# ruizhecao96/CMGAN

Measured on NVIDIA H100. Metric: utterances/sec (2 s @16 kHz) generator fwd+bwd, higher is better.
Workload: dtype tf32

## Files before the change

cmgan_b200/_lib.py:

```python
from __future__ import annotations

import ctypes
import os
import re

HERE = os.path.dirname(os.path.abspath(__file__))
ROOT = os.path.dirname(HERE)
HEADER = os.path.join(ROOT, "include", "cmgan_b200.h")
LIB_PATH = os.path.join(HERE, "libcmgan_b200.so")
MAX_TAPS = 16


class GemmArgs(ctypes.Structure):
    _fields_ = [
        ("A", ctypes.c_void_p), ("lda", ctypes.c_longlong),
        ("B", ctypes.c_void_p), ("sb_tap", ctypes.c_longlong), ("sb_k", ctypes.c_longlong), ("sb_n", ctypes.c_longlong),
        ("bias", ctypes.c_void_p),
        ("C", ctypes.c_void_p), ("ldc", ctypes.c_longlong),
        ("M", ctypes.c_int), ("N", ctypes.c_int), ("Cin", ctypes.c_int), ("ntaps", ctypes.c_int),
        ("conv", ctypes.c_int), ("OH", ctypes.c_int), ("OW", ctypes.c_int), ("IH", ctypes.c_int), ("IW", ctypes.c_int),
        ("mul_y", ctypes.c_int), ("mul_x", ctypes.c_int), ("div_y", ctypes.c_int), ("div_x", ctypes.c_int),
        ("dy", ctypes.c_int * MAX_TAPS), ("dx", ctypes.c_int * MAX_TAPS),
        ("tap_off", ctypes.c_longlong * MAX_TAPS),
        ("pro", ctypes.c_int), ("pro_alpha", ctypes.c_float), ("p0", ctypes.c_void_p), ("p1", ctypes.c_void_p), ("p2", ctypes.c_void_p),
        ("rows_per_batch", ctypes.c_longlong), ("pstride", ctypes.c_longlong),
        ("epi", ctypes.c_int), ("alpha", ctypes.c_float), ("R", ctypes.c_void_p), ("ldr", ctypes.c_longlong),
        ("aux", ctypes.c_void_p), ("ldaux", ctypes.c_longlong), ("e0", ctypes.c_void_p), ("e1", ctypes.c_void_p),
        ("seed", ctypes.c_ulonglong), ("drop_thr", ctypes.c_uint), ("inv_keep", ctypes.c_float),
        ("pro_seed", ctypes.c_ulonglong), ("pro_thr", ctypes.c_uint), ("pro_inv_keep", ctypes.c_float),
        ("D", ctypes.c_void_p), ("ldd", ctypes.c_longlong), ("prod", ctypes.c_int), ("dbias", ctypes.c_void_p),
        ("precision", ctypes.c_int),
        ("ws", ctypes.c_void_p), ("ws_floats", ctypes.c_longlong),
        ("C2", ctypes.c_void_p), ("ldc2", ctypes.c_longlong),
        ("seed_dev", ctypes.c_void_p),
        ("b_packed", ctypes.c_int),
    ]


_CTYPE = {
    "int": ctypes.c_int, "long long": ctypes.c_longlong, "unsigned long long": ctypes.c_ulonglong,
    "unsigned int": ctypes.c_uint, "float": ctypes.c_float, "double": ctypes.c_double,
}


def parse_header(path: str = HEADER):
    protos = {}
    pat = re.compile(r"^\s*(const char\*|int|long long)\s+(cmgan_\w+)\((.*)\);\s*$")
    with open(path) as fh:
        for line in fh:
            m = pat.match(line)
            if not m:
# ... 47 lines not shown
```

cmgan_b200/csrc/gemm_args.h:

```cpp
#pragma once
#include <stdint.h>

#define CMGAN_MAX_TAPS 16

enum CmganPro {
    CMGAN_PRO_NONE = 0,
    CMGAN_PRO_LN = 1,
    CMGAN_PRO_SWISH_DROP = 2,
    CMGAN_PRO_BN_SWISH = 3,
    CMGAN_PRO_DROP = 4,
    CMGAN_PRO_IN_PRELU = 5
};
enum CmganEpi {
    CMGAN_EPI_NONE = 0,
    CMGAN_EPI_DROP_RES = 1,
    CMGAN_EPI_DSWISH_DROP = 2,
    CMGAN_EPI_DBNSWISH = 3,
    CMGAN_EPI_ACC = 4,
    CMGAN_EPI_SWISH_DUAL = 5
};

typedef struct CmganGemmArgs {
    const float* A; long long lda;
    const float* B; long long sb_tap, sb_k, sb_n;
// ... 3 lines not shown
    int conv, OH, OW, IH, IW, mul_y, mul_x, div_y, div_x;
    int dy[CMGAN_MAX_TAPS], dx[CMGAN_MAX_TAPS];
    long long tap_off[CMGAN_MAX_TAPS];
    int pro; float pro_alpha; const float* p0; const float* p1; const float* p2; long long rows_per_batch; long long pstride;
    int epi; float alpha; const float* R; long long ldr; const float* aux; long long ldaux; const float* e0; const float* e1;
    unsigned long long seed; unsigned int drop_thr; float inv_keep;
    unsigned long long pro_seed; unsigned int pro_thr; float pro_inv_keep;
    const float* D; long long ldd; int prod; float* dbias;
    int precision;
    float* ws; long long ws_floats;
    float* C2; long long ldc2;
    const unsigned long long* seed_dev;
    int b_packed;
} CmganGemmArgs;

typedef struct CmganPackDesc {
    const float* src; float* dst; long long sb_tap, sb_k, sb_n; long long Cin, ntaps, N;
} CmganPackDesc;
```

cmgan_b200/csrc/gemm_tc.cu:

```cuda
#include <cuda.h>

#include "common.cuh"
#include "../../include/cmgan_b200.h"
#include "gemm_device.cuh"
#include "tc_ptx.cuh"

namespace {
using namespace cmgan_gemm;
using namespace cmgan_tc;

constexpr int BM = 64;
constexpr int KC = 32;
constexpr int A_STAGE_BYTES = BM * KC * 4;
constexpr int NPROD = 128;
constexpr int NTHREADS = 256;
constexpr int SLAB = 64;
constexpr int STG_LD = SLAB + 4;
constexpr int STG_BYTES = 4 * 16 * STG_LD * 4;
constexpr int SMEM_LIMIT = 227 * 1024;
constexpr int SMEM_LIMIT2 = 112 * 1024;
constexpr int RESIDENT_MAX = 96 * 1024;

__global__ void pack_b_kernel(const float* __restrict__ B, long sb_tap, long sb_k, long sb_n, int Cin, int ntaps, int N, int BN,
                              float* __restrict__ out) {
    long total = (long)ntaps * (Cin / KC) * BN * KC;
    long i = (long)blockIdx.x * blockDim.x + threadIdx.x;
    if (i >= total) return;
    int kk = (int)(i % KC); long t = i / KC; int n = (int)(t % BN); long chunk = t / BN;
    int cpt = Cin / KC;
    int tap = (int)(chunk / cpt), kc = (int)(chunk % cpt);
    float v = 0.f;
    if (n < N) v = to_tf32(__ldg(B + (long)tap * sb_tap + (long)(kc * KC + kk) * sb_k + (long)n * sb_n));
    int c = kk >> 2, j = kk & 3;
// ... 3 lines not shown
__global__ void pack_all_kernel(const CmganPackDesc* __restrict__ descs) {
    const CmganPackDesc d = descs[blockIdx.y];
    const int Cin = (int)d.Cin, N = (int)d.N;
    const long total = d.ntaps * (Cin / KC) * (long)N * KC;
    for (long i = (long)blockIdx.x * blockDim.x + threadIdx.x; i < total; i += (long)gridDim.x * blockDim.x) {
        int kk = (int)(i % KC); long t = i / KC; int n = (int)(t % N); long chunk = t / N;
        int cpt = Cin / KC;
        int tap = (int)(chunk / cpt), kc = (int)(chunk % cpt);
        float v = to_tf32(__ldg(d.src + (long)tap * d.sb_tap + (long)(kc * KC + kk) * d.sb_k + (long)n * d.sb_n));
        int c = kk >> 2, j = kk & 3;
        d.dst[(chunk * N + n) * KC + ((c ^ (n & 7)) << 2) + j] = v;
    }
}

struct TcCfg { int BN, stages, resident, ntiles, tma, nfx, nty, W, H; };
constexpr int PW = 8, PH = 8;

struct TileRing { uint32_t sA, sB, bars; int stages, b_tile_bytes, nchunks, resident, lane; };

template <int NB, int NBMAX>
__device__ __forceinline__ void tile_mma(float (&acc)[NBMAX][8], const TileRing& r, long& q) {
    auto empty_bar = [&](long qq) { return r.bars + 8u * (r.stages + (int)(qq % r.stages)); };
    for (int ch = 0; ch < r.nchunks; ++ch, ++q) {
        const int s = (int)(q % r.stages);
        const uint32_t par = (uint32_t)((q / r.stages) & 1);
        mbar_wait(r.bars + 8u * s, par);
        const uint64_t adesc = gmma_desc_sw128(r.sA + s * A_STAGE_BYTES);
        const uint64_t bdesc = gmma_desc_sw128(r.sB + (r.resident ? ch : s) * r.b_tile_bytes);
        wgmma_fence();
        mma_chunk<NB, NBMAX>(acc, adesc, bdesc, ch == 0);
        wgmma_commit();
        wgmma_wait<1>();
        if (ch > 0) {
            __syncwarp();
            if (r.lane == 0) mbar_arrive(empty_bar(q - 1));
        }
    }
    wgmma_wait<0>();
    __syncwarp();
    if (r.lane == 0) mbar_arrive(empty_bar(q - 1));
}
template <int NBMAX, int I = 1>
__device__ __forceinline__ void tile_mma_nw(int nw, float (&acc)[NBMAX][8], const TileRing& r, long& q) {
    if constexpr (4 * I <= NBMAX) {
        if (nw == I) tile_mma<4 * I, NBMAX>(acc, r, q);
        else tile_mma_nw<NBMAX, I + 1>(nw, acc, r, q);
    }
}

template <bool ASYNC_A, int NBMAX, int EPI, bool PATCH>
__global__ void __launch_bounds__(NTHREADS, NBMAX == 4 ? 2 : 1) gemm_rows_tc_kernel(const __grid_constant__ CmganGemmArgs g, const float* __restrict__ Bp,
                                                                                  const TcCfg cfg, const __grid_constant__ CUtensorMap tmA) {
    extern __shared__ uint8_t smem_raw[];
    const uint32_t base = (smem_u32(smem_raw) + 1023u) & ~1023u;
    uint8_t* base_ptr = smem_raw + (base - smem_u32(smem_raw));
    const int BN = cfg.BN, stages = cfg.stages;
    const int b_tile_bytes = BN * KC * 4;
    const int cpt = g.Cin / KC;
    const int nchunks = cpt * g.ntaps;
    const uint32_t sA = base;
    const uint32_t sB = sA + stages * A_STAGE_BYTES;
    const uint32_t b_region = (uint32_t)(cfg.resident ? nchunks : stages) * b_tile_bytes;
    const uint32_t sStg = sB + b_region;
    const uint32_t bars = sStg + STG_BYTES;
    auto full_bar = [&](int s) { return bars + 8u * s; };
    auto empty_bar = [&](int s) { return bars + 8u * (stages + s); };
    const uint32_t bready_bar = bars + 8u * (2 * stages);

    const int tid = threadIdx.x, warp = tid >> 5, lane = tid & 31;
    const int ntiles = cfg.ntiles;
    const int my_tiles = (ntiles - (int)blockIdx.x + (int)gridDim.x - 1) / (int)gridDim.x;

    if (tid == 0) {
        for (int s = 0; s < stages; ++s) { mbar_init(full_bar(s), cfg.tma ? 1 : NPROD + (cfg.resident ? 0 : 1)); mbar_init(empty_bar(s), 4); }
        mbar_init(bready_bar, 1);
        fence_barrier_init();
    }
    __syncthreads();

    if (warp < 4) {
        const int c = tid & 7;
        const int rr = tid >> 3;
        uint32_t dst_off[4];
#pragma unroll
        for (int i = 0; i < 4; ++i) { const int r = rr + 16 * i; dst_off[i] = r * 128 + ((c ^ (r & 7)) << 4); }
        const long total = (long)my_tiles * nchunks;
        if (tid == 0 && cfg.resident) {
            mbar_arrive_expect_tx(bready_bar, (uint32_t)(nchunks * b_tile_bytes));
            for (int ch = 0; ch < nchunks; ++ch)
                bulk_g2s(sB + ch * b_tile_bytes, Bp + (long)ch * BN * KC, (uint32_t)b_tile_bytes, bready_bar);
        }
#define B_STAGE(q, s)                                                                                                    \
        if (tid == 0 && !cfg.resident) {                                                                                 \
            if (!cfg.tma) mbar_arrive_expect_tx(full_bar(s), (uint32_t)b_tile_bytes);                                    \
            bulk_g2s(sB + (s) * b_tile_bytes, Bp + (long)((q) % nchunks) * BN * KC, (uint32_t)b_tile_bytes, full_bar(s)); \
        }

        if (ASYNC_A && cfg.tma) {
            if (tid == 0) {
                for (long q = 0; q < total; ++q) {
                    const int lt = (int)(q / nchunks), ch = (int)(q - (long)lt * nchunks);
                    const int s = (int)(q % stages);
                    const uint32_t par = (uint32_t)((q / stages) & 1);
                    mbar_wait(empty_bar(s), par ^ 1u);
                    mbar_arrive_expect_tx(full_bar(s), (uint32_t)(A_STAGE_BYTES + (cfg.resident ? 0 : b_tile_bytes)));
                    B_STAGE(q, s)
                    const int tile = blockIdx.x + lt * gridDim.x;
                    if (!PATCH) {
                        tma_load_2d(sA + s * A_STAGE_BYTES, &tmA, ch * KC, tile * BM, full_bar(s));
                    } else {
                        const int fx = tile % cfg.nfx, ty = (tile / cfg.nfx) % cfg.nty, bimg = tile / (cfg.nfx * cfg.nty);
                        const int tap = ch / cpt, kc = ch - tap * cpt;
                        tma_load_4d(sA + s * A_STAGE_BYTES, &tmA, kc * KC, fx * PW + g.dx[tap], ty * PH + g.dy[tap], bimg, full_bar(s));
                    }
                }
            }
            __syncwarp();
        } else if (ASYNC_A) {
            const int LAG = stages >= 4 ? 2 : 1;
            long rowoff[4];
            RowInfo ri[4];
            int cur_tile = -1, cur_tap = -1;
            for (long q = 0; q < total + LAG; ++q) {
                if (q < total) {
                    const int lt = (int)(q / nchunks), ch = (int)(q - (long)lt * nchunks);
                    const int s = (int)(q % stages);
                    const uint32_t par = (uint32_t)((q / stages) & 1);
                    const int tap = ch / cpt, k0 = (ch - tap * cpt) * KC + c * 4;
                    if (lt != cur_tile) {
                        cur_tile = lt; cur_tap = -1;
                        const int m0 = (blockIdx.x + lt * gridDim.x) * BM;
#pragma unroll
                        for (int i = 0; i < 4; ++i) ri[i] = decode_row(g, m0 + rr + 16 * i);
                    }
                    if (tap != cur_tap) {
                        cur_tap = tap;
#pragma unroll
                        for (int i = 0; i < 4; ++i) {
                            long r = in_row_of(g, ri[i], tap);
                            rowoff[i] = r < 0 ? -1 : g.tap_off[tap] + r * g.lda;
                        }
                    }
                    mbar_wait(empty_bar(s), par ^ 1u);
                    B_STAGE(q, s)
                    const uint32_t sbase = sA + s * A_STAGE_BYTES;
#pragma unroll
                    for (int i = 0; i < 4; ++i) {
                        const bool ok = rowoff[i] >= 0;
                        cp_async16(sbase + dst_off[i], g.A + (ok ? rowoff[i] + k0 : 0), ok ? 16u : 0u);
                    }
                }
                cp_async_commit();
                const long done = q - LAG;
                if (done >= 0) {
                    if (LAG == 2) cp_async_wait<2>(); else cp_async_wait<1>();
                    fence_proxy_async();
                    mbar_arrive(full_bar((int)(done % stages)));
                }
            }
        } else {
            float mean[4], rstd[4];
            RowInfo ri[4];
            int cur_tile = -1;
            for (long q = 0; q < total; ++q) {
                const int lt = (int)(q / nchunks), ch = (int)(q - (long)lt * nchunks);
                const int s = (int)(q % stages);
                const uint32_t par = (uint32_t)((q / stages) & 1);
                const int tap = ch / cpt, k0 = (ch - tap * cpt) * KC + c * 4;
                if (lt != cur_tile) {
                    cur_tile = lt;
                    const int m0 = (blockIdx.x + lt * gridDim.x) * BM;
#pragma unroll
                    for (int i = 0; i < 4; ++i) {
                        ri[i] = decode_row(g, m0 + rr + 16 * i);
                        mean[i] = 0.f; rstd[i] = 1.f;
                        if (g.pro == CMGAN_PRO_LN) {
                            long r = in_row_of(g, ri[i], 0);
                            if (r >= 0) { float2 st = __ldg(reinterpret_cast<const float2*>(g.p0) + r); mean[i] = st.x; rstd[i] = st.y; }
                        }
                    }
                }
                ChunkParams cp;
                load_chunk_params(g, k0, cp);
                float4 v[4];
                long rows[4];
#pragma unroll
                for (int i = 0; i < 4; ++i) {
                    rows[i] = in_row_of(g, ri[i], tap);
                    v[i] = rows[i] >= 0 ? __ldg(reinterpret_cast<const float4*>(g.A + g.tap_off[tap] + rows[i] * g.lda + k0)) : make_float4(0.f, 0.f, 0.f, 0.f);
                }
#pragma unroll
                for (int i = 0; i < 4; ++i)
                    if (rows[i] >= 0) v[i] = transform4(g, v[i], rows[i], k0, mean[i], rstd[i], cp);
                mbar_wait(empty_bar(s), par ^ 1u);
                B_STAGE(q, s)
                const uint32_t sbase = sA + s * A_STAGE_BYTES;
#pragma unroll
                for (int i = 0; i < 4; ++i)
                    asm volatile("st.shared.v4.f32 [%0], {%1, %2, %3, %4};" ::"r"(sbase + dst_off[i]), "f"(to_tf32(v[i].x)), "f"(to_tf32(v[i].y)),
                                 "f"(to_tf32(v[i].z)), "f"(to_tf32(v[i].w)) : "memory");
                fence_proxy_async();
                mbar_arrive(full_bar(s));
            }
        }
#undef B_STAGE
    } else {
        const int cw = warp - 4;
        const int nb = BN / 16;
        float acc[NBMAX][8];
#pragma unroll
        for (int j = 0; j < NBMAX; ++j)
#pragma unroll
            for (int i = 0; i < 8; ++i) acc[j][i] = 0.f;
        float* stg = reinterpret_cast<float*>(base_ptr + (sStg - base)) + cw * 16 * STG_LD;
        const int col4 = (lane & 15) * 4;
        const int rsub = lane >> 4;
        const int fg = lane >> 2, ft = lane & 3;
        constexpr bool DROPS = EPI == CMGAN_EPI_DROP_RES || EPI == CMGAN_EPI_DSWISH_DROP || EPI == CMGAN_EPI_SWISH_DUAL;
        const uint32_t seed32 = DROPS ? cmgan_seed32(eff_seed(g)) : 0u;
        const uint32_t thr16 = g.drop_thr >> 16;
        const bool drop_on = DROPS && g.drop_thr != 0u;
        constexpr bool patch = PATCH;
        const float inv_keep = g.inv_keep, alpha = g.alpha;
        const float* xbase = nullptr;
        long ldx = 0;
        if (EPI == CMGAN_EPI_DROP_RES) { xbase = g.R; ldx = g.ldr; }
        else if (EPI == CMGAN_EPI_DSWISH_DROP || EPI == CMGAN_EPI_DBNSWISH) { xbase = g.aux; ldx = g.ldaux; }
        else if (EPI == CMGAN_EPI_ACC) { xbase = g.C; ldx = g.ldc; }
        if (cfg.resident) mbar_wait(bready_bar, 0);
        const TileRing ring{sA, sB, bars, stages, b_tile_bytes, nchunks, cfg.resident, lane};
        long q = 0;
        for (int lt = 0; lt < my_tiles; ++lt) {
            tile_mma_nw<NBMAX>((nb + 3) / 4, acc, ring, q);
            const int tile = blockIdx.x + lt * gridDim.x;
            long mfirst;
            int hi_rows, vhi, vlo;
            if (patch) {
                const int fx = tile % cfg.nfx, ty = (tile / cfg.nfx) % cfg.nty, bimg = tile / (cfg.nfx * cfg.nty);
                const int y0 = ty * PH + cw * 2, x0 = fx * PW;
                mfirst = ((long)bimg * cfg.H + y0) * cfg.W + x0 + rsub;
                hi_rows = cfg.W; vhi = cfg.H - y0; vlo = cfg.W - x0;
            } else {
                const int mrow0 = tile * BM + cw * 16;
                mfirst = (long)mrow0 + rsub;
                hi_rows = 8; vhi = 2; vlo = g.M - mrow0;
            }
            auto row_ok = [&](int ps) { return patch ? ((ps >> 2) < vhi && 2 * (ps & 3) + rsub < vlo) : (2 * ps + rsub < vlo); };
            auto row_delta = [&](int ps) { return (long)(ps >> 2) * hi_rows + 2 * (ps & 3); };
            const bool any_row = row_ok(0);
#pragma unroll
            for (int sl = 0; sl < NBMAX / 4; ++sl) {
                const int n0 = sl * SLAB;
                if (n0 >= BN) break;
                const int ncols = min(SLAB, BN - n0);
#pragma unroll
                for (int jj = 0; jj < 4; ++jj) {
                    if (16 * jj >= ncols) break;
                    const float* d = acc[4 * sl + jj];
// ... 92 lines not shown
using PFN_encodeTiled = CUresult (*)(CUtensorMap*, CUtensorMapDataType, cuuint32_t, void*, const cuuint64_t*, const cuuint64_t*, const cuuint32_t*,
                                      const cuuint32_t*, CUtensorMapInterleave, CUtensorMapSwizzle, CUtensorMapL2promotion, CUtensorMapFloatOOBfill);
PFN_encodeTiled get_encoder() {
    static PFN_encodeTiled encode = nullptr;
    static bool tried = false;
    if (!tried) {
        tried = true;
        void* fn = nullptr;
        cudaDriverEntryPointQueryResult qres;
        if (cudaGetDriverEntryPoint("cuTensorMapEncodeTiled", &fn, cudaEnableDefault, &qres) == cudaSuccess && qres == cudaDriverEntryPointSuccess)
            encode = reinterpret_cast<PFN_encodeTiled>(fn);
    }
    return encode;
}

template <bool ASYNC_A, int NBMAX, int EPI, bool PATCH = false>
int launch_variant(const CmganGemmArgs& a, const TcCfg& cfg, int grid, size_t smem, cudaStream_t st, const CUtensorMap& tm) {
    static bool attr_set = false;
    if (!attr_set) {
        cudaError_t e = cudaFuncSetAttribute(gemm_rows_tc_kernel<ASYNC_A, NBMAX, EPI, PATCH>, cudaFuncAttributeMaxDynamicSharedMemorySize, SMEM_LIMIT);
        if (e != cudaSuccess) { cmgan_set_error("gemm_rows_tc: cudaFuncSetAttribute: %s", cudaGetErrorString(e)); return -1; }
        attr_set = true;
    }
    gemm_rows_tc_kernel<ASYNC_A, NBMAX, EPI, PATCH><<<grid, NTHREADS, smem, st>>>(a, a.ws, cfg, tm);
    return 0;
}

}

int cmgan_gemm_rows_tc_launch(const CmganGemmArgs* a, cudaStream_t st) {
    if (!tc_supported(a)) return 1;
    TcCfg cfg;
    cfg.BN = a->N;
    const int b_tile = cfg.BN * KC * 4;
    const int nchunks = (a->Cin / KC) * a->ntaps;
    cfg.resident = (long)nchunks * b_tile <= RESIDENT_MAX ? 1 : 0;
    const int resident_bytes = cfg.resident ? nchunks * b_tile : 0;
    const int per_stage = A_STAGE_BYTES + (cfg.resident ? 0 : b_tile);
    const int fixed = 1024  + STG_BYTES + 256  + resident_bytes;
    const int ctas = (a->pro == CMGAN_PRO_NONE && cfg.BN <= 64 && fixed + 3 * per_stage <= SMEM_LIMIT2) ? 2 : 1;
    const bool narrow = ctas == 2;
    cfg.stages = ((ctas == 2 ? SMEM_LIMIT2 : SMEM_LIMIT) - fixed) / per_stage;
    if (cfg.stages > 8) cfg.stages = 8;
    if (cfg.stages < 2) return 1;
    cfg.ntiles = cdiv(a->M, BM);
    const size_t smem = (size_t)fixed + (size_t)cfg.stages * per_stage;
    if (g_num_sms == 0) {
        int dev = 0;
        cudaGetDevice(&dev);
        cudaDeviceGetAttribute(&g_num_sms, cudaDevAttrMultiProcessorCount, dev);
    }
    alignas(64) CUtensorMap tm;
    memset(&tm, 0, sizeof(tm));
    cfg.tma = 0;
    cfg.nfx = cfg.nty = 1; cfg.W = cfg.H = 0;
    if (a->pro == CMGAN_PRO_NONE && !a->conv && a->ntaps == 1 && a->lda % 4 == 0) {
        PFN_encodeTiled encode = get_encoder();
        if (encode) {
            const cuuint64_t gdim[2] = {(cuuint64_t)a->Cin, (cuuint64_t)a->M};
            const cuuint64_t gstride[1] = {(cuuint64_t)a->lda * sizeof(float)};
            const cuuint32_t box[2] = {(cuuint32_t)KC, (cuuint32_t)BM};
            const cuuint32_t estr[2] = {1, 1};
            CUresult r = encode(&tm, CU_TENSOR_MAP_DATA_TYPE_FLOAT32, 2, const_cast<float*>(a->A + a->tap_off[0]), gdim, gstride, box, estr,
                                CU_TENSOR_MAP_INTERLEAVE_NONE, CU_TENSOR_MAP_SWIZZLE_128B, CU_TENSOR_MAP_L2_PROMOTION_L2_256B,
                                CU_TENSOR_MAP_FLOAT_OOB_FILL_NONE);
            if (r == CUDA_SUCCESS) cfg.tma = 1;
        }
    }
    bool same_off = true;
    for (int t = 1; t < a->ntaps; ++t) same_off = same_off && a->tap_off[t] == a->tap_off[0];
    if (a->pro == CMGAN_PRO_NONE && (a->epi == CMGAN_EPI_NONE || a->epi == CMGAN_EPI_ACC) && a->conv && a->mul_y == 1 && a->mul_x == 1 && a->div_y == 1 && a->div_x == 1 && a->OH == a->IH &&
        a->OW == a->IW && same_off && a->M % ((long long)a->OH * a->OW) == 0) {
        PFN_encodeTiled encode = get_encoder();
        if (encode) {
            const long long Bn = a->M / ((long long)a->OH * a->OW);
            const cuuint64_t gdim[4] = {(cuuint64_t)a->Cin, (cuuint64_t)a->IW, (cuuint64_t)a->IH, (cuuint64_t)Bn};
            const cuuint64_t gstride[3] = {(cuuint64_t)a->lda * sizeof(float), (cuuint64_t)a->IW * a->lda * sizeof(float),
                                           (cuuint64_t)a->IH * a->IW * a->lda * sizeof(float)};
            const cuuint32_t box[4] = {(cuuint32_t)KC, (cuuint32_t)PW, (cuuint32_t)PH, 1};
            const cuuint32_t estr[4] = {1, 1, 1, 1};
            CUresult r = encode(&tm, CU_TENSOR_MAP_DATA_TYPE_FLOAT32, 4, const_cast<float*>(a->A + a->tap_off[0]), gdim, gstride, box, estr,
                                CU_TENSOR_MAP_INTERLEAVE_NONE, CU_TENSOR_MAP_SWIZZLE_128B, CU_TENSOR_MAP_L2_PROMOTION_L2_256B,
                                CU_TENSOR_MAP_FLOAT_OOB_FILL_NONE);
            const long long nfx = cdiv(a->OW, PW), nty = cdiv(a->OH, PH);
            if (r == CUDA_SUCCESS && Bn * nfx * nty < (1ll << 30)) {
                cfg.tma = 2; cfg.nfx = (int)nfx; cfg.nty = (int)nty; cfg.W = a->OW; cfg.H = a->OH;
                cfg.ntiles = (int)(Bn * nfx * nty);
            }
        }
    }
    if (a->pro == CMGAN_PRO_NONE && cfg.tma == 0 && cfg.stages < 3) return 1;
    if (!a->b_packed) {
        long total = (long)nchunks * cfg.BN * KC;
        pack_b_kernel<<<cdiv(total, 256), 256, 0, st>>>(a->B, a->sb_tap, a->sb_k, a->sb_n, a->Cin, a->ntaps, a->N, cfg.BN, a->ws);
        if (cmgan_check_launch("pack_b_kernel")) return -1;
    }
    const int grid = cfg.ntiles < ctas * g_num_sms ? cfg.ntiles : ctas * g_num_sms;
    const int variant = a->pro != CMGAN_PRO_NONE ? 0 : (narrow ? 1 : 2);
    int rc = -2;
#define CMGAN_TC_LAUNCH(E)                                                                                            \
    case E:                                                                                                           \
        rc = variant == 0   ? launch_variant<false, 16, E>(*a, cfg, grid, smem, st, tm)                               \
             : variant == 1 ? launch_variant<true, 4, E>(*a, cfg, grid, smem, st, tm)                                 \
                            : launch_variant<true, 16, E>(*a, cfg, grid, smem, st, tm);                               \
        break;
    if (cfg.tma == 2) {
        if (a->epi == CMGAN_EPI_NONE)
            rc = narrow ? launch_variant<true, 4, CMGAN_EPI_NONE, true>(*a, cfg, grid, smem, st, tm)
                        : launch_variant<true, 16, CMGAN_EPI_NONE, true>(*a, cfg, grid, smem, st, tm);
        else
            rc = narrow ? launch_variant<true, 4, CMGAN_EPI_ACC, true>(*a, cfg, grid, smem, st, tm)
                        : launch_variant<true, 16, CMGAN_EPI_ACC, true>(*a, cfg, grid, smem, st, tm);
    } else
    switch (a->epi) {
        CMGAN_TC_LAUNCH(CMGAN_EPI_NONE)
        CMGAN_TC_LAUNCH(CMGAN_EPI_DROP_RES)
        CMGAN_TC_LAUNCH(CMGAN_EPI_DSWISH_DROP)
        CMGAN_TC_LAUNCH(CMGAN_EPI_DBNSWISH)
        CMGAN_TC_LAUNCH(CMGAN_EPI_ACC)
        CMGAN_TC_LAUNCH(CMGAN_EPI_SWISH_DUAL)
        default: break;
    }
#undef CMGAN_TC_LAUNCH
    if (rc == -2) { cmgan_set_error("gemm_rows_tc: unknown epilogue %d", a->epi); return -1; }
    if (rc) return -1;
    return cmgan_check_launch("gemm_rows_tc_kernel");
}

CMGAN_API int cmgan_pack_weight(const float* src, float* dst, long long sb_tap, long long sb_k, long long sb_n, int Cin, int ntaps, int N, void* stream) {
    CMGAN_REQUIRE(src && dst && Cin > 0 && Cin % KC == 0 && ntaps >= 1 && N > 0, "cmgan_pack_weight: bad arguments (Cin must be a multiple of %d)", KC);
    const long total = (long)ntaps * Cin * N;
    pack_b_kernel<<<cdiv(total, 256), 256, 0, (cudaStream_t)stream>>>(src, sb_tap, sb_k, sb_n, Cin, ntaps, N, N, dst);
    return cmgan_check_launch("pack_b_kernel");
}

CMGAN_API int cmgan_pack_weights(const CmganPackDesc* descs, int n, void* stream) {
    CMGAN_REQUIRE(descs || n == 0, "cmgan_pack_weights: null table");
    if (n == 0) return 0;
    pack_all_kernel<<<dim3(48, n), 256, 0, (cudaStream_t)stream>>>(descs);
    return cmgan_check_launch("pack_all_kernel");
}
```

cmgan_b200/csrc/tc_ptx.cuh:

```cuda
#pragma once
#include "common.cuh"

namespace cmgan_tc {

__device__ __forceinline__ uint32_t smem_u32(const void* p) { return (uint32_t)__cvta_generic_to_shared(p); }

__device__ __forceinline__ void mbar_init(uint32_t bar, uint32_t count) {
    asm volatile("mbarrier.init.shared::cta.b64 [%0], %1;" ::"r"(bar), "r"(count) : "memory");
}
__device__ __forceinline__ void mbar_arrive(uint32_t bar) {
    asm volatile("mbarrier.arrive.shared::cta.b64 _, [%0];" ::"r"(bar) : "memory");
}
__device__ __forceinline__ void mbar_arrive_expect_tx(uint32_t bar, uint32_t bytes) {
    asm volatile("mbarrier.arrive.expect_tx.shared::cta.b64 _, [%0], %1;" ::"r"(bar), "r"(bytes) : "memory");
}
__device__ __forceinline__ void mbar_wait(uint32_t bar, uint32_t parity) {
    uint32_t done = 0;
    for (uint32_t spin = 0; !done; ++spin) {
        asm volatile("{\n\t.reg .pred p;\n\tmbarrier.try_wait.parity.shared::cta.b64 p, [%1], %2;\n\tselp.u32 %0, 1, 0, p;\n\t}"
                     : "=r"(done) : "r"(bar), "r"(parity) : "memory");
        if (spin > (1u << 28)) __trap();
    }
}
__device__ __forceinline__ bool mbar_test(uint32_t bar, uint32_t parity) {
// ... 33 lines not shown

__device__ __forceinline__ float to_tf32(float x) {
    uint32_t r;
    asm("cvt.rna.tf32.f32 %0, %1;" : "=r"(r) : "f"(x));
    return __uint_as_float(r);
}

__device__ __forceinline__ uint64_t gmma_desc_sw128(uint32_t saddr) {
    uint64_t d = 0;
    d |= (uint64_t)((saddr & 0x3FFFF) >> 4);
    d |= (uint64_t)1 << 16;
    d |= (uint64_t)(1024 >> 4) << 32;
    d |= (uint64_t)1 << 62;
    return d;
}
__device__ __forceinline__ void wgmma_fence() { asm volatile("wgmma.fence.sync.aligned;" ::: "memory"); }
__device__ __forceinline__ void wgmma_commit() { asm volatile("wgmma.commit_group.sync.aligned;" ::: "memory"); }
template <int N>
__device__ __forceinline__ void wgmma_wait() { asm volatile("wgmma.wait_group.sync.aligned %0;" ::"n"(N) : "memory"); }
__device__ __forceinline__ void wgmma_m64n16k8_tf32(float d[8], uint64_t adesc, uint64_t bdesc, uint32_t accumulate) {
    asm volatile("{\n\t.reg .pred p;\n\tsetp.ne.b32 p, %10, 0;\n\t"
                 "wgmma.mma_async.sync.aligned.m64n16k8.f32.tf32.tf32 {%0, %1, %2, %3, %4, %5, %6, %7}, %8, %9, p, 1, 1;\n\t}"
                 : "+f"(d[0]), "+f"(d[1]), "+f"(d[2]), "+f"(d[3]), "+f"(d[4]), "+f"(d[5]), "+f"(d[6]), "+f"(d[7])
                 : "l"(adesc), "l"(bdesc), "r"(accumulate));
}
#define CMGAN_D8(b) "+f"(d[b][0]), "+f"(d[b][1]), "+f"(d[b][2]), "+f"(d[b][3]), "+f"(d[b][4]), "+f"(d[b][5]), "+f"(d[b][6]), "+f"(d[b][7])
__device__ __forceinline__ void wgmma_m64n64k8_tf32(float (&d)[4][8], uint64_t adesc, uint64_t bdesc, uint32_t accumulate) {
    asm volatile("{\n\t.reg .pred p;\n\tsetp.ne.b32 p, %34, 0;\n\t"
                 "wgmma.mma_async.sync.aligned.m64n64k8.f32.tf32.tf32 "
                 "{%0, %1, %2, %3, %4, %5, %6, %7, %8, %9, %10, %11, %12, %13, %14, %15, "
// ... 77 lines not shown
```

include/cmgan_b200.h:

```cpp
#ifndef CMGAN_B200_H
#define CMGAN_B200_H
#include "../cmgan_b200/csrc/gemm_args.h"

#ifdef __cplusplus
extern "C" {
#endif

const char* cmgan_last_error(void);
int cmgan_abi_version(void);
int cmgan_gemm_args_size(void);
int cmgan_set_tf32_rounding(int on);

int cmgan_gemm_rows_f32(const CmganGemmArgs* a, void* stream);
int cmgan_gemm_wgrad_f32(const CmganGemmArgs* a, void* stream);
int cmgan_pack_weights(const CmganPackDesc* descs, int n, void* stream);
int cmgan_pack_weight(const float* src, float* dst, long long sb_tap, long long sb_k, long long sb_n, int Cin, int ntaps, int N, void* stream);



int cmgan_ffn_fwd(const float* x, long long ldx, long long M, const float* ln_g, const float* ln_b, const float* W1p, const float* b1, const float* W2p, const float* b2, float alpha, unsigned long long seed1, unsigned long long seed2, unsigned int thr, float inv_keep, const unsigned long long* seed_dev, float* out, long long ldo, void* stream);
int cmgan_ffn_bwd(const float* x, long long ldx, const float* dz, long long lddz, const float* dout, long long lddo, const float* res2, long long ldr2, long long M, const float* ln_g, const float* ln_b, const float* W1p, const float* b1, const float* W2tp, const float* W1tp, unsigned long long seed1, unsigned int thr, float inv_keep, const unsigned long long* seed_dev, float* dx, long long lddx, float* a_out, float* dh_out, float* xn_out, float* dgamma, float* dbeta, float* ws, void* stream);

int cmgan_ln_stats(const float* x, long long ldx, long long M, float* stats, void* stream);
int cmgan_ln_apply(const float* x, long long ldx, long long M, const float* gamma, const float* beta, const float* res, long long ldr, float* y, long long ldy, float* stats, int round_tf32, void* stream);
int cmgan_ln_bwd(const float* dy, long long lddy, const float* x, long long ldx, const float* stats, const float* gamma, long long M, const float* res, long long ldr, const float* res2, long long ldr2, float* dx, long long lddx, float* dgamma, float* dbeta, void* stream);
int cmgan_ln_bwd_drop(const float* dy, long long lddy, const float* x, long long ldx, const float* stats, const float* gamma, long long M, const float* res, long long ldr, const float* res2, long long ldr2, float* dx, long long lddx, float* dgamma, float* dbeta, float* dz, long long lddz, float alpha, unsigned long long seed, unsigned int thr, float inv_keep, const unsigned long long* seed_dev, void* stream);
int cmgan_norm_stats(const float* x, long long ldx, int G, long long rows_per_group, int C, double* sums, void* stream);
int cmgan_norm_finalize(const double* sums, long long n, int G, int C, int mode, const float* gamma, const float* beta, float* running_mean, float* running_var, float momentum, float* scale, float* shift, float* mean_out, float* rstd_out, long long tstride, void* stream);
int cmgan_norm_bwd_reduce(const float* x, long long ldx, const float* dact, long long ldd, int G, long long rows_per_group, int C, int act, const float* scale, const float* shift, const float* mean, const float* rstd, long long tstride, const float* slope, double* S, float* dslope, void* stream);
// ... 119 lines not shown
```

Measured before the change: 95.17.

## Use two consumer warpgroups per CTA with 128-row tiles and register rebalancing

Doubles the row-GEMM tile from 64 to 128 rows by adding a second consumer warpgroup that shares each staged B tile, with producers loading both halves per stage. setmaxnreg moves registers from the producer warpgroup to the consumers, and patch tiles grow to 8x16. The point is to reuse each B chunk over more rows and cut per-tile overhead. In exchange, the CTA gets larger and uses more shared memory per stage, which can leave fewer pipeline stages, fewer tiles in flight and worse tail balance on small layers. Plan selection is also factored into a make_plan function exposed to Python.

Measured after the change: 98.41, median of 6. 1.03x the previous value.

```diff
diff --git a/cmgan_b200/_lib.py b/cmgan_b200/_lib.py
--- a/cmgan_b200/_lib.py
+++ b/cmgan_b200/_lib.py
@@ -35,6 +35,23 @@
         ("seed_dev", ctypes.c_void_p),
         ("b_packed", ctypes.c_int),
     ]
+
+
+class GemmRowsPlan(ctypes.Structure):
+    _fields_ = [(n, ctypes.c_int) for n in (
+        "supported", "mode", "tile_rows", "consumers", "threads", "ctas_per_sm", "stages", "resident", "nchunks", "b_tile_bytes",
+        "smem_bytes", "producer_regs", "consumer_regs", "entry_regs", "patch_w", "patch_h")] + [("ntiles", ctypes.c_longlong)]
+
+
+ROWS_MODES = ("register", "cp.async", "tma2d", "patch")
+
+
+def gemm_rows_plan(args: GemmArgs) -> dict:
+    p = GemmRowsPlan()
+    lib().call("cmgan_gemm_rows_tc_plan", ctypes.byref(args), ctypes.byref(p))
+    d = {n: getattr(p, n) for n, _ in GemmRowsPlan._fields_}
+    d["mode"] = ROWS_MODES[p.mode]
+    return d
 
 
 _CTYPE = {
diff --git a/cmgan_b200/csrc/gemm_args.h b/cmgan_b200/csrc/gemm_args.h
--- a/cmgan_b200/csrc/gemm_args.h
+++ b/cmgan_b200/csrc/gemm_args.h
@@ -41,6 +41,24 @@
     int b_packed;
 } CmganGemmArgs;
 
+enum CmganRowsMode {
+    CMGAN_ROWS_REGISTER = 0,
+    CMGAN_ROWS_CPASYNC = 1,
+    CMGAN_ROWS_TMA2D = 2,
+    CMGAN_ROWS_PATCH = 3
+};
+typedef struct CmganGemmRowsPlan {
+    int supported;
+    int mode;
+    int tile_rows, consumers, threads, ctas_per_sm;
+    int stages, resident, nchunks, b_tile_bytes;
+    int smem_bytes;
+    int producer_regs, consumer_regs;
+    int entry_regs;
+    int patch_w, patch_h;
+    long long ntiles;
+} CmganGemmRowsPlan;
+
 typedef struct CmganPackDesc {
     const float* src; float* dst; long long sb_tap, sb_k, sb_n; long long Cin, ntaps, N;
 } CmganPackDesc;
diff --git a/cmgan_b200/csrc/gemm_tc.cu b/cmgan_b200/csrc/gemm_tc.cu
--- a/cmgan_b200/csrc/gemm_tc.cu
+++ b/cmgan_b200/csrc/gemm_tc.cu
@@ -10,13 +10,21 @@
 using namespace cmgan_tc;
 
 constexpr int BM = 64;
+constexpr int NCONS = 2;
+constexpr int TILE_M = NCONS * BM;
 constexpr int KC = 32;
-constexpr int A_STAGE_BYTES = BM * KC * 4;
+constexpr int A_HALF_BYTES = BM * KC * 4;
 constexpr int NPROD = 128;
-constexpr int NTHREADS = 256;
 constexpr int SLAB = 64;
 constexpr int STG_LD = SLAB + 4;
-constexpr int STG_BYTES = 4 * 16 * STG_LD * 4;
+template <int NC> struct TileShape {
+    static constexpr int rows = NC * BM, stage_bytes = NC * A_HALF_BYTES, threads = NPROD + NC * 128;
+    static constexpr int rows_per_thread = rows / (NPROD / 8), stg_bytes = NC * 4 * 16 * STG_LD * 4;
+};
+constexpr int ENTRY_REGS = 168;
+template <bool ASYNC_A> struct RegSplit { static constexpr int prod = ASYNC_A ? 72 : 120, cons = ASYNC_A ? 216 : 192; };
+static_assert(128 * RegSplit<true>::prod + 256 * RegSplit<true>::cons <= TileShape<2>::threads * ENTRY_REGS, "register split");
+static_assert(128 * RegSplit<false>::prod + 256 * RegSplit<false>::cons <= TileShape<2>::threads * ENTRY_REGS, "register split");
 constexpr int SMEM_LIMIT = 227 * 1024;
 constexpr int SMEM_LIMIT2 = 112 * 1024;
 constexpr int RESIDENT_MAX = 96 * 1024;
@@ -50,9 +58,10 @@
 }
 
 struct TcCfg { int BN, stages, resident, ntiles, tma, nfx, nty, W, H; };
-constexpr int PW = 8, PH = 8;
-
-struct TileRing { uint32_t sA, sB, bars; int stages, b_tile_bytes, nchunks, resident, lane; };
+constexpr int PW = 8, PH = 16;
+static_assert(PW * PH == TILE_M, "a patch tile is one tile");
+
+struct TileRing { uint32_t sA, sB, bars; int stages, a_stage_bytes, b_tile_bytes, nchunks, resident, lane; };
 
 template <int NB, int NBMAX>
 __device__ __forceinline__ void tile_mma(float (&acc)[NBMAX][8], const TileRing& r, long& q) {
@@ -61,7 +70,7 @@
         const int s = (int)(q % r.stages);
         const uint32_t par = (uint32_t)((q / r.stages) & 1);
         mbar_wait(r.bars + 8u * s, par);
-        const uint64_t adesc = gmma_desc_sw128(r.sA + s * A_STAGE_BYTES);
+        const uint64_t adesc = gmma_desc_sw128(r.sA + s * r.a_stage_bytes);
         const uint64_t bdesc = gmma_desc_sw128(r.sB + (r.resident ? ch : s) * r.b_tile_bytes);
         wgmma_fence();
         mma_chunk<NB, NBMAX>(acc, adesc, bdesc, ch == 0);
@@ -84,9 +93,11 @@
     }
 }
 
-template <bool ASYNC_A, int NBMAX, int EPI, bool PATCH>
-__global__ void __launch_bounds__(NTHREADS, NBMAX == 4 ? 2 : 1) gemm_rows_tc_kernel(const __grid_constant__ CmganGemmArgs g, const float* __restrict__ Bp,
-                                                                                  const TcCfg cfg, const __grid_constant__ CUtensorMap tmA) {
+template <bool ASYNC_A, int NBMAX, int EPI, bool PATCH, int NC>
+__global__ void __launch_bounds__(TileShape<NC>::threads, NC == 1 ? 2 : 1) gemm_rows_tc_kernel(const __grid_constant__ CmganGemmArgs g, const float* __restrict__ Bp,
+                                                                 const TcCfg cfg, const __grid_constant__ CUtensorMap tmA) {
+    static_assert(NC == 2 || (ASYNC_A && !PATCH && NBMAX == 4), "64-row tiles only for the narrow cp.async plan");
+    using TS = TileShape<NC>;
     extern __shared__ uint8_t smem_raw[];
     const uint32_t base = (smem_u32(smem_raw) + 1023u) & ~1023u;
     uint8_t* base_ptr = smem_raw + (base - smem_u32(smem_raw));
@@ -95,10 +106,10 @@
     const int cpt = g.Cin / KC;
     const int nchunks = cpt * g.ntaps;
     const uint32_t sA = base;
-    const uint32_t sB = sA + stages * A_STAGE_BYTES;
+    const uint32_t sB = sA + stages * TS::stage_bytes;
     const uint32_t b_region = (uint32_t)(cfg.resident ? nchunks : stages) * b_tile_bytes;
     const uint32_t sStg = sB + b_region;
-    const uint32_t bars = sStg + STG_BYTES;
+    const uint32_t bars = sStg + TS::stg_bytes;
     auto full_bar = [&](int s) { return bars + 8u * s; };
     auto empty_bar = [&](int s) { return bars + 8u * (stages + s); };
     const uint32_t bready_bar = bars + 8u * (2 * stages);
@@ -108,18 +119,17 @@
     const int my_tiles = (ntiles - (int)blockIdx.x + (int)gridDim.x - 1) / (int)gridDim.x;
 
     if (tid == 0) {
-        for (int s = 0; s < stages; ++s) { mbar_init(full_bar(s), cfg.tma ? 1 : NPROD + (cfg.resident ? 0 : 1)); mbar_init(empty_bar(s), 4); }
+        for (int s = 0; s < stages; ++s) { mbar_init(full_bar(s), cfg.tma ? 1 : NPROD + (cfg.resident ? 0 : 1)); mbar_init(empty_bar(s), 4 * NC); }
         mbar_init(bready_bar, 1);
         fence_barrier_init();
     }
     __syncthreads();
 
     if (warp < 4) {
+        if constexpr (NC == 2) setmaxnreg_dec<RegSplit<ASYNC_A>::prod>();
         const int c = tid & 7;
         const int rr = tid >> 3;
-        uint32_t dst_off[4];
-#pragma unroll
-        for (int i = 0; i < 4; ++i) { const int r = rr + 16 * i; dst_off[i] = r * 128 + ((c ^ (r & 7)) << 4); }
+        const uint32_t dst_off0 = rr * 128 + ((c ^ (rr & 7)) << 4);
         const long total = (long)my_tiles * nchunks;
         if (tid == 0 && cfg.resident) {
             mbar_arrive_expect_tx(bready_bar, (uint32_t)(nchunks * b_tile_bytes));
@@ -139,23 +149,23 @@
                     const int s = (int)(q % stages);
                     const uint32_t par = (uint32_t)((q / stages) & 1);
                     mbar_wait(empty_bar(s), par ^ 1u);
-                    mbar_arrive_expect_tx(full_bar(s), (uint32_t)(A_STAGE_BYTES + (cfg.resident ? 0 : b_tile_bytes)));
+                    mbar_arrive_expect_tx(full_bar(s), (uint32_t)(TS::stage_bytes + (cfg.resident ? 0 : b_tile_bytes)));
                     B_STAGE(q, s)
                     const int tile = blockIdx.x + lt * gridDim.x;
                     if (!PATCH) {
-                        tma_load_2d(sA + s * A_STAGE_BYTES, &tmA, ch * KC, tile * BM, full_bar(s));
+                        tma_load_2d(sA + s * TS::stage_bytes, &tmA, ch * KC, tile * TS::rows, full_bar(s));
                     } else {
                         const int fx = tile % cfg.nfx, ty = (tile / cfg.nfx) % cfg.nty, bimg = tile / (cfg.nfx * cfg.nty);
                         const int tap = ch / cpt, kc = ch - tap * cpt;
-                        tma_load_4d(sA + s * A_STAGE_BYTES, &tmA, kc * KC, fx * PW + g.dx[tap], ty * PH + g.dy[tap], bimg, full_bar(s));
+                        tma_load_4d(sA + s * TS::stage_bytes, &tmA, kc * KC, fx * PW + g.dx[tap], ty * PH + g.dy[tap], bimg, full_bar(s));
                     }
                 }
             }
             __syncwarp();
         } else if (ASYNC_A) {
             const int LAG = stages >= 4 ? 2 : 1;
-            long rowoff[4];
-            RowInfo ri[4];
+            long rowoff[TS::rows_per_thread];
+            RowInfo ri[TS::rows_per_thread];
             int cur_tile = -1, cur_tap = -1;
             for (long q = 0; q < total + LAG; ++q) {
                 if (q < total) {
@@ -165,25 +175,25 @@
                     const int tap = ch / cpt, k0 = (ch - tap * cpt) * KC + c * 4;
                     if (lt != cur_tile) {
                         cur_tile = lt; cur_tap = -1;
-                        const int m0 = (blockIdx.x + lt * gridDim.x) * BM;
-#pragma unroll
-                        for (int i = 0; i < 4; ++i) ri[i] = decode_row(g, m0 + rr + 16 * i);
+                        const int m0 = (blockIdx.x + lt * gridDim.x) * TS::rows;
+#pragma unroll
+                        for (int i = 0; i < TS::rows_per_thread; ++i) ri[i] = decode_row(g, m0 + rr + 16 * i);
                     }
                     if (tap != cur_tap) {
                         cur_tap = tap;
 #pragma unroll
-                        for (int i = 0; i < 4; ++i) {
+                        for (int i = 0; i < TS::rows_per_thread; ++i) {
                             long r = in_row_of(g, ri[i], tap);
                             rowoff[i] = r < 0 ? -1 : g.tap_off[tap] + r * g.lda;
                         }
                     }
                     mbar_wait(empty_bar(s), par ^ 1u);
                     B_STAGE(q, s)
-                    const uint32_t sbase = sA + s * A_STAGE_BYTES;
-#pragma unroll
-                    for (int i = 0; i < 4; ++i) {
+                    const uint32_t sbase = sA + s * TS::stage_bytes + dst_off0;
+#pragma unroll
+                    for (int i = 0; i < TS::rows_per_thread; ++i) {
                         const bool ok = rowoff[i] >= 0;
-                        cp_async16(sbase + dst_off[i], g.A + (ok ? rowoff[i] + k0 : 0), ok ? 16u : 0u);
+                        cp_async16(sbase + i * 16 * 128, g.A + (ok ? rowoff[i] + k0 : 0), ok ? 16u : 0u);
                     }
                 }
                 cp_async_commit();
@@ -195,8 +205,8 @@
                 }
             }
         } else {
-            float mean[4], rstd[4];
-            RowInfo ri[4];
+            float mean[TS::rows_per_thread], rstd[TS::rows_per_thread];
+            RowInfo ri[TS::rows_per_thread];
             int cur_tile = -1;
             for (long q = 0; q < total; ++q) {
                 const int lt = (int)(q / nchunks), ch = (int)(q - (long)lt * nchunks);
@@ -205,9 +215,9 @@
                 const int tap = ch / cpt, k0 = (ch - tap * cpt) * KC + c * 4;
                 if (lt != cur_tile) {
                     cur_tile = lt;
-                    const int m0 = (blockIdx.x + lt * gridDim.x) * BM;
-#pragma unroll
-                    for (int i = 0; i < 4; ++i) {
+                    const int m0 = (blockIdx.x + lt * gridDim.x) * TS::rows;
+#pragma unroll
+                    for (int i = 0; i < TS::rows_per_thread; ++i) {
                         ri[i] = decode_row(g, m0 + rr + 16 * i);
                         mean[i] = 0.f; rstd[i] = 1.f;
                         if (g.pro == CMGAN_PRO_LN) {
@@ -218,30 +228,37 @@
                 }
                 ChunkParams cp;
                 load_chunk_params(g, k0, cp);
-                float4 v[4];
-                long rows[4];
-#pragma unroll
-                for (int i = 0; i < 4; ++i) {
-                    rows[i] = in_row_of(g, ri[i], tap);
-                    v[i] = rows[i] >= 0 ? __ldg(reinterpret_cast<const float4*>(g.A + g.tap_off[tap] + rows[i] * g.lda + k0)) : make_float4(0.f, 0.f, 0.f, 0.f);
-                }
-#pragma unroll
-                for (int i = 0; i < 4; ++i)
-                    if (rows[i] >= 0) v[i] = transform4(g, v[i], rows[i], k0, mean[i], rstd[i], cp);
-                mbar_wait(empty_bar(s), par ^ 1u);
-                B_STAGE(q, s)
-                const uint32_t sbase = sA + s * A_STAGE_BYTES;
-#pragma unroll
-                for (int i = 0; i < 4; ++i)
-                    asm volatile("st.shared.v4.f32 [%0], {%1, %2, %3, %4};" ::"r"(sbase + dst_off[i]), "f"(to_tf32(v[i].x)), "f"(to_tf32(v[i].y)),
-                                 "f"(to_tf32(v[i].z)), "f"(to_tf32(v[i].w)) : "memory");
+                const uint32_t sbase = sA + s * TS::stage_bytes + dst_off0;
+#pragma unroll
+                for (int h = 0; h < NC; ++h) {
+                    float4 v[4];
+                    long rows[4];
+#pragma unroll
+                    for (int i = 0; i < 4; ++i) {
+                        rows[i] = in_row_of(g, ri[4 * h + i], tap);
+                        v[i] = rows[i] >= 0 ? __ldg(reinterpret_cast<const float4*>(g.A + g.tap_off[tap] + rows[i] * g.lda + k0)) : make_float4(0.f, 0.f, 0.f, 0.f);
+                    }
+#pragma unroll
+                    for (int i = 0; i < 4; ++i)
+                        if (rows[i] >= 0) v[i] = transform4(g, v[i], rows[i], k0, mean[4 * h + i], rstd[4 * h + i], cp);
+                    if (h == 0) {
+                        mbar_wait(empty_bar(s), par ^ 1u);
+                        B_STAGE(q, s)
+                    }
+#pragma unroll
+                    for (int i = 0; i < 4; ++i)
+                        asm volatile("st.shared.v4.f32 [%0], {%1, %2, %3, %4};" ::"r"(sbase + (4 * h + i) * 16 * 128), "f"(to_tf32(v[i].x)),
+                                     "f"(to_tf32(v[i].y)), "f"(to_tf32(v[i].z)), "f"(to_tf32(v[i].w)) : "memory");
+                }
                 fence_proxy_async();
                 mbar_arrive(full_bar(s));
             }
         }
 #undef B_STAGE
     } else {
+        if constexpr (NC == 2) setmaxnreg_inc<RegSplit<ASYNC_A>::cons>();
         const int cw = warp - 4;
+        const int cons = cw >> 2;
         const int nb = BN / 16;
         float acc[NBMAX][8];
 #pragma unroll
@@ -264,7 +281,7 @@
         else if (EPI == CMGAN_EPI_DSWISH_DROP || EPI == CMGAN_EPI_DBNSWISH) { xbase = g.aux; ldx = g.ldaux; }
         else if (EPI == CMGAN_EPI_ACC) { xbase = g.C; ldx = g.ldc; }
         if (cfg.resident) mbar_wait(bready_bar, 0);
-        const TileRing ring{sA, sB, bars, stages, b_tile_bytes, nchunks, cfg.resident, lane};
+        const TileRing ring{sA + cons * A_HALF_BYTES, sB, bars, stages, TS::stage_bytes, b_tile_bytes, nchunks, cfg.resident, lane};
         long q = 0;
         for (int lt = 0; lt < my_tiles; ++lt) {
             tile_mma_nw<NBMAX>((nb + 3) / 4, acc, ring, q);
@@ -277,7 +294,7 @@
                 mfirst = ((long)bimg * cfg.H + y0) * cfg.W + x0 + rsub;
                 hi_rows = cfg.W; vhi = cfg.H - y0; vlo = cfg.W - x0;
             } else {
-                const int mrow0 = tile * BM + cw * 16;
+                const int mrow0 = tile * TS::rows + cw * 16;
                 mfirst = (long)mrow0 + rsub;
                 hi_rows = 8; vhi = 2; vlo = g.M - mrow0;
             }
@@ -400,37 +417,79 @@
     return encode;
 }
 
-template <bool ASYNC_A, int NBMAX, int EPI, bool PATCH = false>
+void make_plan(const CmganGemmArgs* a, CmganGemmRowsPlan* p) {
+    memset(p, 0, sizeof(*p));
+    if (!tc_supported(a)) return;
+    bool same_off = true;
+    for (int t = 1; t < a->ntaps; ++t) same_off = same_off && a->tap_off[t] == a->tap_off[0];
+    const long long img = (long long)a->OH * a->OW;
+    if (a->pro != CMGAN_PRO_NONE) {
+        p->mode = CMGAN_ROWS_REGISTER;
+    } else if ((a->epi == CMGAN_EPI_NONE || a->epi == CMGAN_EPI_ACC) && a->conv && a->mul_y == 1 && a->mul_x == 1 && a->div_y == 1 &&
+               a->div_x == 1 && a->OH == a->IH && a->OW == a->IW && same_off && img > 0 && a->M % img == 0 &&
+               a->M / img * cdiv((long long)a->OW, (long long)PW) * cdiv((long long)a->OH, (long long)PH) < (1ll << 30)) {
+        p->mode = CMGAN_ROWS_PATCH;
+    } else if (!a->conv && a->ntaps == 1) {
+        p->mode = CMGAN_ROWS_TMA2D;
+    } else {
+        p->mode = CMGAN_ROWS_CPASYNC;
+    }
+    p->b_tile_bytes = a->N * KC * 4;
+    p->nchunks = (a->Cin / KC) * a->ntaps;
+    p->resident = (long)p->nchunks * p->b_tile_bytes <= RESIDENT_MAX ? 1 : 0;
+    const int resident_bytes = p->resident ? p->nchunks * p->b_tile_bytes : 0;
+    const int b_stage = p->resident ? 0 : p->b_tile_bytes;
+    const int fixed1 = 1024  + TileShape<1>::stg_bytes + 256  + resident_bytes;
+    const bool narrow = p->mode == CMGAN_ROWS_CPASYNC && a->N <= 64 && fixed1 + 3 * (TileShape<1>::stage_bytes + b_stage) <= SMEM_LIMIT2;
+    const int nc = narrow ? 1 : 2;
+    p->tile_rows = narrow ? TileShape<1>::rows : TileShape<2>::rows;
+    p->consumers = nc;
+    p->threads = narrow ? TileShape<1>::threads : TileShape<2>::threads;
+    p->ctas_per_sm = narrow ? 2 : 1;
+    p->entry_regs = narrow ? 128 : ENTRY_REGS;
+    const int per_stage = (narrow ? TileShape<1>::stage_bytes : TileShape<2>::stage_bytes) + b_stage;
+    const int fixed = narrow ? fixed1 : 1024 + TileShape<2>::stg_bytes + 256 + resident_bytes;
+    p->stages = ((narrow ? SMEM_LIMIT2 : SMEM_LIMIT) - fixed) / per_stage;
+    if (p->stages > 8) p->stages = 8;
+    p->smem_bytes = fixed + p->stages * per_stage;
+    p->ntiles = cdiv((long long)a->M, (long long)p->tile_rows);
+    if (p->mode == CMGAN_ROWS_PATCH) {
+        p->patch_w = PW;
+        p->patch_h = PH;
+        p->ntiles = a->M / img * cdiv((long long)a->OW, (long long)PW) * cdiv((long long)a->OH, (long long)PH);
+    }
+    const bool async_a = p->mode != CMGAN_ROWS_REGISTER;
+    p->producer_regs = narrow ? p->entry_regs : async_a ? RegSplit<true>::prod : RegSplit<false>::prod;
+    p->consumer_regs = narrow ? p->entry_regs : async_a ? RegSplit<true>::cons : RegSplit<false>::cons;
+    p->supported = p->stages >= 3 ? 1 : 0;
+}
+
+template <bool ASYNC_A, int NBMAX, int EPI, bool PATCH = false, int NC = 2>
 int launch_variant(const CmganGemmArgs& a, const TcCfg& cfg, int grid, size_t smem, cudaStream_t st, const CUtensorMap& tm) {
     static bool attr_set = false;
     if (!attr_set) {
-        cudaError_t e = cudaFuncSetAttribute(gemm_rows_tc_kernel<ASYNC_A, NBMAX, EPI, PATCH>, cudaFuncAttributeMaxDynamicSharedMemorySize, SMEM_LIMIT);
+        cudaError_t e = cudaFuncSetAttribute(gemm_rows_tc_kernel<ASYNC_A, NBMAX, EPI, PATCH, NC>, cudaFuncAttributeMaxDynamicSharedMemorySize, SMEM_LIMIT);
         if (e != cudaSuccess) { cmgan_set_error("gemm_rows_tc: cudaFuncSetAttribute: %s", cudaGetErrorString(e)); return -1; }
         attr_set = true;
     }
-    gemm_rows_tc_kernel<ASYNC_A, NBMAX, EPI, PATCH><<<grid, NTHREADS, smem, st>>>(a, a.ws, cfg, tm);
+    gemm_rows_tc_kernel<ASYNC_A, NBMAX, EPI, PATCH, NC><<<grid, TileShape<NC>::threads, smem, st>>>(a, a.ws, cfg, tm);
     return 0;
 }
 
 }
 
 int cmgan_gemm_rows_tc_launch(const CmganGemmArgs* a, cudaStream_t st) {
-    if (!tc_supported(a)) return 1;
+    CmganGemmRowsPlan p;
+    make_plan(a, &p);
+    if (!p.supported) return 1;
     TcCfg cfg;
     cfg.BN = a->N;
-    const int b_tile = cfg.BN * KC * 4;
-    const int nchunks = (a->Cin / KC) * a->ntaps;
-    cfg.resident = (long)nchunks * b_tile <= RESIDENT_MAX ? 1 : 0;
-    const int resident_bytes = cfg.resident ? nchunks * b_tile : 0;
-    const int per_stage = A_STAGE_BYTES + (cfg.resident ? 0 : b_tile);
-    const int fixed = 1024  + STG_BYTES + 256  + resident_bytes;
-    const int ctas = (a->pro == CMGAN_PRO_NONE && cfg.BN <= 64 && fixed + 3 * per_stage <= SMEM_LIMIT2) ? 2 : 1;
-    const bool narrow = ctas == 2;
-    cfg.stages = ((ctas == 2 ? SMEM_LIMIT2 : SMEM_LIMIT) - fixed) / per_stage;
-    if (cfg.stages > 8) cfg.stages = 8;
-    if (cfg.stages < 2) return 1;
-    cfg.ntiles = cdiv(a->M, BM);
-    const size_t smem = (size_t)fixed + (size_t)cfg.stages * per_stage;
+    cfg.stages = p.stages;
+    cfg.resident = p.resident;
+    cfg.ntiles = (int)cdiv(a->M, TILE_M);
+    if (p.tile_rows != TILE_M) cfg.ntiles = (int)p.ntiles;
+    cfg.tma = 0;
+    cfg.nfx = cfg.nty = 1; cfg.W = cfg.H = 0;
     if (g_num_sms == 0) {
         int dev = 0;
         cudaGetDevice(&dev);
@@ -438,25 +497,19 @@
     }
     alignas(64) CUtensorMap tm;
     memset(&tm, 0, sizeof(tm));
-    cfg.tma = 0;
-    cfg.nfx = cfg.nty = 1; cfg.W = cfg.H = 0;
-    if (a->pro == CMGAN_PRO_NONE && !a->conv && a->ntaps == 1 && a->lda % 4 == 0) {
+    if (p.mode == CMGAN_ROWS_TMA2D) {
         PFN_encodeTiled encode = get_encoder();
         if (encode) {
             const cuuint64_t gdim[2] = {(cuuint64_t)a->Cin, (cuuint64_t)a->M};
             const cuuint64_t gstride[1] = {(cuuint64_t)a->lda * sizeof(float)};
-            const cuuint32_t box[2] = {(cuuint32_t)KC, (cuuint32_t)BM};
+            const cuuint32_t box[2] = {(cuuint32_t)KC, (cuuint32_t)TILE_M};
             const cuuint32_t estr[2] = {1, 1};
             CUresult r = encode(&tm, CU_TENSOR_MAP_DATA_TYPE_FLOAT32, 2, const_cast<float*>(a->A + a->tap_off[0]), gdim, gstride, box, estr,
                                 CU_TENSOR_MAP_INTERLEAVE_NONE, CU_TENSOR_MAP_SWIZZLE_128B, CU_TENSOR_MAP_L2_PROMOTION_L2_256B,
                                 CU_TENSOR_MAP_FLOAT_OOB_FILL_NONE);
             if (r == CUDA_SUCCESS) cfg.tma = 1;
         }
-    }
-    bool same_off = true;
-    for (int t = 1; t < a->ntaps; ++t) same_off = same_off && a->tap_off[t] == a->tap_off[0];
-    if (a->pro == CMGAN_PRO_NONE && (a->epi == CMGAN_EPI_NONE || a->epi == CMGAN_EPI_ACC) && a->conv && a->mul_y == 1 && a->mul_x == 1 && a->div_y == 1 && a->div_x == 1 && a->OH == a->IH &&
-        a->OW == a->IW && same_off && a->M % ((long long)a->OH * a->OW) == 0) {
+    } else if (p.mode == CMGAN_ROWS_PATCH) {
         PFN_encodeTiled encode = get_encoder();
         if (encode) {
             const long long Bn = a->M / ((long long)a->OH * a->OW);
@@ -468,35 +521,29 @@
             CUresult r = encode(&tm, CU_TENSOR_MAP_DATA_TYPE_FLOAT32, 4, const_cast<float*>(a->A + a->tap_off[0]), gdim, gstride, box, estr,
                                 CU_TENSOR_MAP_INTERLEAVE_NONE, CU_TENSOR_MAP_SWIZZLE_128B, CU_TENSOR_MAP_L2_PROMOTION_L2_256B,
                                 CU_TENSOR_MAP_FLOAT_OOB_FILL_NONE);
-            const long long nfx = cdiv(a->OW, PW), nty = cdiv(a->OH, PH);
-            if (r == CUDA_SUCCESS && Bn * nfx * nty < (1ll << 30)) {
-                cfg.tma = 2; cfg.nfx = (int)nfx; cfg.nty = (int)nty; cfg.W = a->OW; cfg.H = a->OH;
-                cfg.ntiles = (int)(Bn * nfx * nty);
+            if (r == CUDA_SUCCESS) {
+                cfg.tma = 2; cfg.nfx = (int)cdiv(a->OW, PW); cfg.nty = (int)cdiv(a->OH, PH); cfg.W = a->OW; cfg.H = a->OH;
+                cfg.ntiles = (int)p.ntiles;
             }
         }
     }
-    if (a->pro == CMGAN_PRO_NONE && cfg.tma == 0 && cfg.stages < 3) return 1;
     if (!a->b_packed) {
-        long total = (long)nchunks * cfg.BN * KC;
+        long total = (long)p.nchunks * cfg.BN * KC;
         pack_b_kernel<<<cdiv(total, 256), 256, 0, st>>>(a->B, a->sb_tap, a->sb_k, a->sb_n, a->Cin, a->ntaps, a->N, cfg.BN, a->ws);
         if (cmgan_check_launch("pack_b_kernel")) return -1;
     }
-    const int grid = cfg.ntiles < ctas * g_num_sms ? cfg.ntiles : ctas * g_num_sms;
-    const int variant = a->pro != CMGAN_PRO_NONE ? 0 : (narrow ? 1 : 2);
+    const int grid = cfg.ntiles < p.ctas_per_sm * g_num_sms ? cfg.ntiles : p.ctas_per_sm * g_num_sms;
+    const size_t smem = (size_t)p.smem_bytes;
     int rc = -2;
 #define CMGAN_TC_LAUNCH(E)                                                                                            \
     case E:                                                                                                           \
-        rc = variant == 0   ? launch_variant<false, 16, E>(*a, cfg, grid, smem, st, tm)                               \
-             : variant == 1 ? launch_variant<true, 4, E>(*a, cfg, grid, smem, st, tm)                                 \
-                            : launch_variant<true, 16, E>(*a, cfg, grid, smem, st, tm);                               \
+        rc = a->pro != CMGAN_PRO_NONE ? launch_variant<false, 16, E>(*a, cfg, grid, smem, st, tm)                     \
+             : p.consumers == 1       ? launch_variant<true, 4, E, false, 1>(*a, cfg, grid, smem, st, tm)             \
+                                      : launch_variant<true, 16, E>(*a, cfg, grid, smem, st, tm);                     \
         break;
     if (cfg.tma == 2) {
-        if (a->epi == CMGAN_EPI_NONE)
-            rc = narrow ? launch_variant<true, 4, CMGAN_EPI_NONE, true>(*a, cfg, grid, smem, st, tm)
-                        : launch_variant<true, 16, CMGAN_EPI_NONE, true>(*a, cfg, grid, smem, st, tm);
-        else
-            rc = narrow ? launch_variant<true, 4, CMGAN_EPI_ACC, true>(*a, cfg, grid, smem, st, tm)
-                        : launch_variant<true, 16, CMGAN_EPI_ACC, true>(*a, cfg, grid, smem, st, tm);
+        rc = a->epi == CMGAN_EPI_NONE ? launch_variant<true, 16, CMGAN_EPI_NONE, true>(*a, cfg, grid, smem, st, tm)
+                                      : launch_variant<true, 16, CMGAN_EPI_ACC, true>(*a, cfg, grid, smem, st, tm);
     } else
     switch (a->epi) {
         CMGAN_TC_LAUNCH(CMGAN_EPI_NONE)
@@ -513,6 +560,12 @@
     return cmgan_check_launch("gemm_rows_tc_kernel");
 }
 
+CMGAN_API int cmgan_gemm_rows_tc_plan(const CmganGemmArgs* a, CmganGemmRowsPlan* out) {
+    CMGAN_REQUIRE(a && out, "cmgan_gemm_rows_tc_plan: null argument");
+    make_plan(a, out);
+    return 0;
+}
+
 CMGAN_API int cmgan_pack_weight(const float* src, float* dst, long long sb_tap, long long sb_k, long long sb_n, int Cin, int ntaps, int N, void* stream) {
     CMGAN_REQUIRE(src && dst && Cin > 0 && Cin % KC == 0 && ntaps >= 1 && N > 0, "cmgan_pack_weight: bad arguments (Cin must be a multiple of %d)", KC);
     const long total = (long)ntaps * Cin * N;
diff --git a/cmgan_b200/csrc/tc_ptx.cuh b/cmgan_b200/csrc/tc_ptx.cuh
--- a/cmgan_b200/csrc/tc_ptx.cuh
+++ b/cmgan_b200/csrc/tc_ptx.cuh
@@ -71,6 +71,11 @@
     d |= (uint64_t)1 << 62;
     return d;
 }
+template <int R>
+__device__ __forceinline__ void setmaxnreg_dec() { asm volatile("setmaxnreg.dec.sync.aligned.u32 %0;" ::"n"(R)); }
+template <int R>
+__device__ __forceinline__ void setmaxnreg_inc() { asm volatile("setmaxnreg.inc.sync.aligned.u32 %0;" ::"n"(R)); }
+
 __device__ __forceinline__ void wgmma_fence() { asm volatile("wgmma.fence.sync.aligned;" ::: "memory"); }
 __device__ __forceinline__ void wgmma_commit() { asm volatile("wgmma.commit_group.sync.aligned;" ::: "memory"); }
 template <int N>
diff --git a/include/cmgan_b200.h b/include/cmgan_b200.h
--- a/include/cmgan_b200.h
+++ b/include/cmgan_b200.h
@@ -13,6 +13,7 @@
 
 int cmgan_gemm_rows_f32(const CmganGemmArgs* a, void* stream);
 int cmgan_gemm_wgrad_f32(const CmganGemmArgs* a, void* stream);
+int cmgan_gemm_rows_tc_plan(const CmganGemmArgs* a, CmganGemmRowsPlan* out);
 int cmgan_pack_weights(const CmganPackDesc* descs, int n, void* stream);
 int cmgan_pack_weight(const float* src, float* dst, long long sb_tap, long long sb_k, long long sb_n, int Cin, int ntaps, int N, void* stream);
 
```
